# cloudflare/circl

Hardware: NVIDIA B200
Metric: ML-KEM-768 encaps/sec (higher is better)
Workload: dtype int16

## Files before the change

### circl_b200/csrc/api.cu

```cuda
#include <sched.h>
#include <stdarg.h>
#include <stdlib.h>
#include <string.h>

#include <algorithm>

#include "../../include/circl_b200.h"
#include "common.cuh"
#include "context.h"

#include <sys/mman.h>

namespace cb200 {

static thread_local char g_err[512] = "";
void set_error(const char* fmt, ...) {
  va_list ap;
  va_start(ap, fmt);
  vsnprintf(g_err, sizeof g_err, fmt, ap);
  va_end(ap);
}

Runtime& rt() {
  static Runtime* r = new Runtime;
  return *r;
}

static thread_local Dev* t_dev = nullptr;
static thread_local WorkSet* t_ws3 = nullptr;
static thread_local cudaStream_t t_stream = nullptr;

Dev& ctx() {
  if (!t_dev) {
    fprintf(stderr, "cb200: internal error: no device bound to this thread\n");
    abort();
  }
  return *t_dev;
}
WorkSet& wset(int slot) {
  if (slot >= 0 && slot < Dev::kSlots) return ctx().staging[slot];
  if (!t_ws3) {
    fprintf(stderr, "cb200: internal error: no work set bound to this thread\n");
    abort();
  }
  return *t_ws3;
}
bool profiling_on() { return rt().profiling; }

static const char* kKernelNames[KID_COUNT] = {
    "kyber_ntt", "kyber_invntt", "kyber_dot", "kyber_elementwise",
    "mlkem_hash_ek", "mlkem_g", "mlkem_sample", "mlkem_encrypt",
    "dil_ntt", "dil_invntt", "dil_dot", "dil_elementwise",
    "mldsa_expand_key", "mldsa_mu_rhoprime", "mldsa_mask", "mldsa_w", "mldsa_challenge", "mldsa_response",
    "mldsa_compact", "x25519", "hybrid_glue", "keccak_f1600", "sampler", "mlkem_sample_fix"};
const char* kernel_name(int id) { return (id >= 0 && id < KID_COUNT) ? kKernelNames[id] : "?"; }

KernelScope::KernelScope(int id_, cudaStream_t st_) : st(st_), id(id_) {
  Runtime& r = rt();
  r.launches.fetch_add(1, std::memory_order_relaxed);
  if (r.profiling) {
    cudaEventCreate(&a);
    cudaEventRecord(a, st);
  }
}
KernelScope::~KernelScope() {
  if (!a) return;
  Runtime& r = rt();
  cudaEvent_t b;
  cudaEventCreate(&b);
  cudaEventRecord(b, st);
  std::lock_guard<std::mutex> lock(r.prof_mu);
  r.prof.push_back(ProfRec{id, a, b});
}

int require_ready() {
  if (!rt().ready) {
    set_error("cb200: not initialised (call cb200_init or cb200_init_devices; there is no CPU fallback)");
    return CB200_ERR_NOT_INIT;
  }
  return 0;
}

bool is_device_ptr(const void* p, int* device) {
  if (!p) return false;
  cudaPointerAttributes a;
  if (cudaPointerGetAttributes(&a, p) != cudaSuccess) {
    cudaGetLastError();
// ... 45 lines not shown
  return 0;
}

int ensure_pinned(size_t bytes, void** out) {
  Dev& c = ctx();
  if (c.pinned_bytes < bytes) {
    if (c.pinned) CB200_CUDA(cudaFreeHost(c.pinned));
    c.pinned = nullptr;
    c.pinned_bytes = 0;
    CB200_CUDA(cudaHostAlloc(&c.pinned, bytes, cudaHostAllocDefault));
    c.pinned_bytes = bytes;
  }
  *out = c.pinned;
  return 0;
}

int ensure_smem_attr(const void* func, int bytes) {
  Dev& c = ctx();
  std::lock_guard<std::mutex> lock(c.attr_mu);
  if (c.attr_done.count(func)) return 0;
  CB200_CUDA(cudaFuncSetAttribute(func, cudaFuncAttributeMaxDynamicSharedMemorySize, bytes));
  c.attr_done.insert(func);
  return 0;
}

static int wset_create(WorkSet& w) {
  CB200_CUDA(cudaEventCreateWithFlags(&w.ev_fork, cudaEventDisableTiming));
  for (int l = 0; l < 2; l++) {
    CB200_CUDA(cudaStreamCreateWithFlags(&w.lane[l], cudaStreamNonBlocking));
    CB200_CUDA(cudaEventCreateWithFlags(&w.ev_join[l], cudaEventDisableTiming));
  }
  CB200_CUDA(cudaStreamCreateWithFlags(&w.copy, cudaStreamNonBlocking));
  CB200_CUDA(cudaEventCreateWithFlags(&w.ev_copy, cudaEventDisableTiming));
  CB200_CUDA(cudaMalloc(&w.small, 256));
  CB200_CUDA(cudaHostAlloc(&w.pin, 64, cudaHostAllocDefault));
  return 0;
}
static void wset_destroy(WorkSet& w) {
  for (int l = 0; l < 2; l++) {
    if (w.fix[l]) cudaFree(w.fix[l]);
    w.fix[l] = nullptr;
    w.fix_bytes[l] = 0;
    if (w.work[l]) cudaFree(w.work[l]);
    w.work[l] = nullptr;
    w.work_bytes[l] = 0;
    if (w.lane[l]) cudaStreamDestroy(w.lane[l]);
    if (w.ev_join[l]) cudaEventDestroy(w.ev_join[l]);
    w.lane[l] = nullptr;
    w.ev_join[l] = nullptr;
  }
  if (w.ev_fork) cudaEventDestroy(w.ev_fork);
  w.ev_fork = nullptr;
  if (w.copy) cudaStreamDestroy(w.copy);
  if (w.ev_copy) cudaEventDestroy(w.ev_copy);
  w.copy = nullptr;
  w.ev_copy = nullptr;
  if (w.small) cudaFree(w.small);
  if (w.pin) cudaFreeHost(w.pin);
  w.small = w.pin = nullptr;
}

static bool local_cpus(int device, cpu_set_t* out) {
  char id[32] = "";
  if (cudaDeviceGetPCIBusId(id, sizeof id, device) != cudaSuccess) {
    cudaGetLastError();
    return false;
  }
  for (char* p = id; *p; p++) *p = (char)tolower(*p);
  char path[128];
  snprintf(path, sizeof path, "/sys/bus/pci/devices/%s/local_cpulist", id);
  FILE* f = fopen(path, "r");
  if (!f) return false;
  char line[1024] = "";
  const bool got = fgets(line, sizeof line, f) != nullptr;
  fclose(f);
  if (!got) return false;
  cpu_set_t allowed;
  CPU_ZERO(&allowed);
  if (sched_getaffinity(0, sizeof allowed, &allowed) != 0) return false;
  CPU_ZERO(out);
  int n = 0;
  for (char* tok = strtok(line, ",\n"); tok; tok = strtok(nullptr, ",\n")) {
    int lo = 0, hi = 0;
    const int k = sscanf(tok, "%d-%d", &lo, &hi);
    if (k < 1) continue;
    if (k == 1) hi = lo;
    for (int c = lo; c <= hi && c < CPU_SETSIZE; c++)
      if (CPU_ISSET(c, &allowed)) {
        CPU_SET(c, out);
// ... 643 lines not shown
```

### circl_b200/csrc/context.h

```cpp
#pragma once
#include <cuda_runtime.h>
#include <stddef.h>
#include <stdint.h>

#include <atomic>
#include <condition_variable>
#include <deque>
#include <functional>
#include <map>
#include <memory>
#include <mutex>
#include <set>
#include <string>
#include <thread>
#include <vector>

#include "launch.h"

namespace cb200 {

struct ProfRec {
  int id;
  cudaEvent_t a, b;
};

struct WorkSet {
  void* work[2] = {nullptr, nullptr};
  size_t work_bytes[2] = {0, 0};
  cudaStream_t lane[2] = {nullptr, nullptr};
  cudaEvent_t ev_fork = nullptr, ev_join[2] = {nullptr, nullptr};
  cudaStream_t copy = nullptr;
  cudaEvent_t ev_copy = nullptr;
  void* fix[2] = {nullptr, nullptr};
  size_t fix_bytes[2] = {0, 0};
  void* small = nullptr;
  void* pin = nullptr;
  std::mutex mu;
};

struct Dev {
  int device = -1;
  int sm_count = 148;
  void* kyber_tw = nullptr;
  void* dil_tw = nullptr;
  void* x25519_table = nullptr;
  static constexpr int kSlots = 4;
  cudaStream_t pipe[kSlots] = {};
  cudaStream_t h2d = nullptr, d2h = nullptr;
  cudaEvent_t ev_in[kSlots] = {}, ev_k[kSlots] = {}, ev_out[kSlots] = {};
  void* scratch[kSlots] = {};
  size_t scratch_bytes[kSlots] = {};
  WorkSet staging[kSlots];
  void* pinned = nullptr;
  size_t pinned_bytes = 0;
  std::mutex sets_mu;
  std::map<cudaStream_t, std::unique_ptr<WorkSet>> sets;
  std::mutex attr_mu;
  std::set<const void*> attr_done;
  std::thread worker;
  std::mutex q_mu;
  std::condition_variable q_cv;
  std::deque<std::function<void()>> q;
  bool stop = false;
};

struct Runtime {
  std::vector<std::unique_ptr<Dev>> devs;
  std::atomic<bool> ready{false};
  std::atomic<uint64_t> launches{0};
  std::atomic<unsigned> next_dev{0};
  bool profiling = false;
  std::vector<ProfRec> prof;
  std::mutex prof_mu;
  std::mutex init_mu;
};
Runtime& rt();

enum KernelId {
  KID_KYBER_NTT = 0, KID_KYBER_INVNTT, KID_KYBER_DOT, KID_KYBER_EW,
  KID_MLKEM_HASH_EK, KID_MLKEM_G, KID_MLKEM_SAMPLE, KID_MLKEM_ENCRYPT,
  KID_DIL_NTT, KID_DIL_INVNTT, KID_DIL_DOT, KID_DIL_EW,
  KID_MLDSA_EXPAND, KID_MLDSA_MU, KID_MLDSA_MASK, KID_MLDSA_W, KID_MLDSA_CHALLENGE, KID_MLDSA_RESPONSE,
  KID_MLDSA_COMPACT, KID_X25519, KID_HYBRID_GLUE, KID_KECCAK, KID_SAMPLER, KID_MLKEM_SAMPLE_FIX, KID_COUNT
};
const char* kernel_name(int id);

Dev& ctx();
constexpr int kDevSlot = Dev::kSlots;
constexpr int kLevel1 = 8;
WorkSet& wset(int slot);
bool profiling_on();

struct KernelScope {
  cudaStream_t st;
  int id;
  cudaEvent_t a = nullptr;
  KernelScope(int id, cudaStream_t st);
  ~KernelScope();
};
int require_ready();
bool is_device_ptr(const void* p, int* device = nullptr);
int ensure_scratch(int slot, size_t bytes);
int ensure_work(int slot, size_t bytes, void** out);
int ensure_pinned(size_t bytes, void** out);
int ensure_fix(int slot, int lane, size_t bytes, cudaStream_t st, void** out);
int ensure_smem_attr(const void* func, int bytes);
inline void count_launch(uint64_t n = 1) { rt().launches.fetch_add(n, std::memory_order_relaxed); }

struct DeviceCall {
  int rc = 0;
  cudaStream_t st = nullptr;
  Dev* dev = nullptr;
  WorkSet* ws = nullptr;
  explicit DeviceCall(const void* any_device_buffer);
  ~DeviceCall();
  DeviceCall(const DeviceCall&) = delete;
// ... 37 lines not shown
```

### circl_b200/csrc/mlkem.cu

```cuda
#include <stdlib.h>
#include <string.h>

#include <algorithm>

#include "../../include/circl_b200.h"
#include "context.h"
#include "mlkem_internal.h"
#include "keccak.cuh"
#include "kyber.cuh"

namespace cb200 {
namespace mlkem {

using kyber::N;
using kyber::Q;

template <int K>
struct Params {
  static constexpr int k = K;
  static constexpr int du = (K == 4) ? 11 : 10;
  static constexpr int dv = (K == 4) ? 5 : 4;
  static constexpr int ek_bytes = 384 * K + 32;
  static constexpr int ct_bytes = 32 * (du * K + dv);
  static constexpr int eta1 = (K == 2) ? 3 : 2;
// ... 75 lines not shown
  }
  return wp;
}

__device__ __forceinline__ uint32_t prmt_sx(uint32_t a, uint32_t b, uint32_t sel) {
  uint32_t d;
  asm("prmt.b32 %0, %1, %2, %3;" : "=r"(d) : "r"(a), "r"(b), "r"(sel));
  return d;
}
__device__ __forceinline__ void cbd2_words(uint32_t t, uint32_t (&w)[4]) {
  const uint32_t d = (t & 0x55555555u) + ((t >> 1) & 0x55555555u);
  const uint32_t ae = d & 0x03030303u, be = (d >> 2) & 0x03030303u;
  const uint32_t ao = (d >> 4) & 0x03030303u, bo = (d >> 6) & 0x03030303u;
  const uint32_t ce = ((ae | 0x80808080u) - be) ^ 0x80808080u;
  const uint32_t co = ((ao | 0x80808080u) - bo) ^ 0x80808080u;
  w[0] = prmt_sx(ce, co, 0xc480);
  w[1] = prmt_sx(ce, co, 0xd591);
  w[2] = prmt_sx(ce, co, 0xe6a2);
  w[3] = prmt_sx(ce, co, 0xf7b3);
}
__device__ __forceinline__ void cbd2_store(const uint64_t (&a)[25], int16_t* __restrict__ dst) {
  uint4* out = reinterpret_cast<uint4*>(dst);
#pragma unroll
  for (int i = 0; i < 16; i++) {
    uint32_t lo[4], hi[4];
    cbd2_words((uint32_t)a[i], lo);
    cbd2_words((uint32_t)(a[i] >> 32), hi);
    out[2 * i] = make_uint4(lo[0], lo[1], lo[2], lo[3]);
    out[2 * i + 1] = make_uint4(hi[0], hi[1], hi[2], hi[3]);
  }
}

constexpr size_t kSub = 8192;
constexpr int kRowWords = 129;
constexpr int kSampleSmem = 128 * kRowWords * 4;

__device__ __forceinline__ void cbd3_store(const uint64_t (&w)[24], int16_t* __restrict__ dst) {
  uint4* out = reinterpret_cast<uint4*>(dst);
#pragma unroll
  for (int g = 0; g < 8; g++) {
    const uint64_t w0 = w[3 * g], w1 = w[3 * g + 1], w2 = w[3 * g + 2];
    uint64_t t[4];
    t[0] = w0;
    t[1] = (w0 >> 48) | (w1 << 16);
    t[2] = (w1 >> 32) | (w2 << 32);
    t[3] = w2 >> 16;
#pragma unroll
    for (int q = 0; q < 4; q++) {
      const uint64_t x = t[q];
      uint64_t d = x & 0x249249249249ull;
      d += (x >> 1) & 0x249249249249ull;
      d += (x >> 2) & 0x249249249249ull;
      uint32_t c[4];
#pragma unroll
      for (int j = 0; j < 4; j++) {
        const int c0 = (int)((d >> (12 * j)) & 7) - (int)((d >> (12 * j + 3)) & 7);
        const int c1 = (int)((d >> (12 * j + 6)) & 7) - (int)((d >> (12 * j + 9)) & 7);
        c[j] = ((uint32_t)c0 & 0xffffu) | ((uint32_t)c1 << 16);
      }
      out[4 * g + q] = make_uint4(c[0], c[1], c[2], c[3]);
    }
  }
}

__device__ __forceinline__ void uniform_stream(uint64_t (&a)[25], uint32_t* row_words) {
  int16_t* row = reinterpret_cast<int16_t*>(row_words);
// ... 320 lines not shown
    t[5] = ((b >> 28) | (c << 4)) & 0xfff;
    t[6] = (c >> 8) & 0xfff;
    t[7] = c >> 20;
#pragma unroll
    for (int j = 0; j < 8; j++) bad |= (t[j] >= (uint32_t)Q);
#pragma unroll
    for (int j = 0; j < 4; j++) aw[4 * g + j] = t[2 * j] | (t[2 * j + 1] << 16);
  }
  return bad;
}

__device__ __forceinline__ uint32_t unpack12_half(const uint32_t (&w)[8], uint32_t (&aw)[8]) {
  uint32_t bad = 0;
#pragma unroll
  for (int g = 0; g < 2; g++) {
    const uint32_t a = w[3 * g], b = w[3 * g + 1], c = w[3 * g + 2];
    uint32_t t[8];
    t[0] = a & 0xfff;
    t[1] = (a >> 12) & 0xfff;
    t[2] = ((a >> 24) | (b << 8)) & 0xfff;
    t[3] = (b >> 4) & 0xfff;
    t[4] = (b >> 16) & 0xfff;
    t[5] = ((b >> 28) | (c << 4)) & 0xfff;
    t[6] = (c >> 8) & 0xfff;
    t[7] = c >> 20;
#pragma unroll
    for (int j = 0; j < 8; j++) bad |= (t[j] >= (uint32_t)Q);
#pragma unroll
    for (int j = 0; j < 4; j++) aw[4 * g + j] = t[2 * j] | (t[2 * j + 1] << 16);
  }
  return bad;
}

template <int K, int THREADS, int MINB>
__global__ void __launch_bounds__(THREADS, MINB) encrypt_dp_kernel(
    const uint8_t* __restrict__ ek, size_t ek_stride, const int16_t* __restrict__ A, int a_shared,
    const int16_t* __restrict__ noise, const uint8_t* __restrict__ m, size_t n, uint8_t* __restrict__ ct,
    uint8_t* __restrict__ ss, uint8_t* __restrict__ status, const kyber::TwPair* __restrict__ tw, int lenient) {
  using P = Params<K>;
  using S = EncSmem<K, THREADS>;
  using namespace kyber;
  constexpr int OCTS = THREADS / 8;
  extern __shared__ __align__(16) uint32_t enc_smem[];
  uint32_t* ops_all = enc_smem;
  uint32_t* tiles = enc_smem + OCTS * S::op_words;
  TwPair* tws = reinterpret_cast<TwPair*>(tiles + OCTS * kPolyWords);
  const int lane = threadIdx.x & 31, warp = threadIdx.x >> 5, oct = lane >> 3, v = lane & 7;
  const unsigned octmask = 0xffu << (8 * oct);
  uint32_t* tile = tiles + (warp * 4 + oct) * kPolyWords;
  uint2* ops = reinterpret_cast<uint2*>(ops_all + (size_t)(warp * 4 + oct) * S::op_words) + v;

  for (int i = threadIdx.x; i < 128; i += THREADS) tws[i] = tw[128 + i];
  __syncthreads();
  const volatile TwLow* tabl = reinterpret_cast<const volatile TwLow*>(tws);
  const size_t base = ((size_t)blockIdx.x * (THREADS / 32) + warp) * 4;
  if (base >= n) return;
  const size_t op_raw = base + oct;
  const bool active = op_raw < n;
  const size_t op = active ? op_raw : n - 1;
  const uint8_t* ekp = ek + op * ek_stride;
  const uint32_t* Ap = reinterpret_cast<const uint32_t*>(A) + (a_shared ? 0 : op * K * K * (N / 2));
  const uint32_t* np = reinterpret_cast<const uint32_t*>(noise) + op * P::n_noise * (N / 2);
  uint8_t* ctp = ct + op * P::ct_bytes;

  int32_t r[32];

  {
    uint32_t nw[16];
#pragma unroll
    for (int q = 0; q < 16; q++) nw[q] = ldg_stream32(np + 8 * q + v);
#pragma unroll 1
    for (int j = 0; j < K; j++) {
#pragma unroll
      for (int q = 0; q < 16; q++) unpack2_lo(nw[q], r[2 * q], r[2 * q + 1]);
      if (j + 1 < K) {
#pragma unroll
        for (int q = 0; q < 16; q++) nw[q] = ldg_stream32(np + (j + 1) * (N / 2) + 8 * q + v);
      }
      fwd_pass_S_lo(r);
      store_S_lo(tile, v, r);
      __syncwarp();
      load_C_lo(tile, v, r);
      fwd_pass_C_lo_smem(r, tabl, v);
      __syncwarp();
#pragma unroll
      for (int q = 0; q < 8; q++) {
        const TwLow z = twl_at(tabl, 64 + 8 * q + v);
#pragma unroll
        for (int h = 0; h < 2; h++) {
          const int blk = 2 * q + h;
          const int32_t b0 = mont_mul_lo(r[2 * blk], kScaleZp, kScaleKk), b1 = mont_mul_lo(r[2 * blk + 1], kScaleZp, kScaleKk);
          int32_t zb1 = mont_mul_lo(b1, z.zp, z.kk);
          if (h) zb1 = -zb1;
          ops[(j * 16 + blk) * 8] = make_uint2(__byte_perm((uint32_t)b0, (uint32_t)zb1, 0x5140),
                                               __byte_perm((uint32_t)b1, (uint32_t)b0, 0x5140));
        }
      }
    }
  }
  __syncwarp();

  auto fetch = [&](int i, int h, int j, uint32_t (&raw)[8]) {
    if (i < K) {
      const uint4* p = reinterpret_cast<const uint4*>(Ap + (i * K + j) * (N / 2) + 16 * v + 8 * h);
      const uint4 x = __ldg(p), y = __ldg(p + 1);
      raw[0] = x.x, raw[1] = x.y, raw[2] = x.z, raw[3] = x.w, raw[4] = y.x, raw[5] = y.y, raw[6] = y.z, raw[7] = y.w;
    } else {
      const uint2* p = reinterpret_cast<const uint2*>(ekp + 384 * j + 48 * v + 24 * h);
      const uint2 x = __ldg(p), y = __ldg(p + 1), z = __ldg(p + 2);
      raw[0] = x.x, raw[1] = x.y, raw[2] = y.x, raw[3] = y.y, raw[4] = z.x, raw[5] = z.y;
    }
  };
  uint32_t bad = 0;
  uint32_t raw[K][8];
#pragma unroll
  for (int j = 0; j < K; j++) fetch(0, 0, j, raw[j]);
#pragma unroll 1
  for (int i = 0; i <= K; i++) {
    uint32_t ew[16];
#pragma unroll 1
    for (int h = 0; h < 2; h++) {
      int32_t p0l[8], p0h[8], p1l[8], p1h[8];
#pragma unroll
      for (int c = 0; c < 8; c++) p0l[c] = p0h[c] = p1l[c] = p1h[c] = 0;
      const int ni = h ? i + 1 : i, nh = h ^ 1;
#pragma unroll
      for (int j = 0; j < K; j++) {
        uint32_t aw[8];
        if (i < K) {
#pragma unroll
          for (int c = 0; c < 8; c++) aw[c] = raw[j][c];
        } else {
          const uint32_t b = unpack12_half(raw[j], aw);
          if (!lenient) bad |= b;
        }
        if (ni <= K) fetch(ni, nh, j, raw[j]);
        const uint2* oj = ops + (size_t)(j * 16 + 8 * h) * 8;
#pragma unroll
        for (int c = 0; c < 8; c++) {
          const uint2 w = oj[c * 8];
          p0l[c] = (int32_t)dp2a_lo_uu(aw[c], w.x, (uint32_t)p0l[c]);
          p0h[c] = dp2a_hi_us(aw[c], w.x, p0h[c]);
          p1l[c] = (int32_t)dp2a_lo_uu(aw[c], w.y, (uint32_t)p1l[c]);
          p1h[c] = dp2a_hi_us(aw[c], w.y, p1h[c]);
        }
      }
      if (h == 0) {
#pragma unroll
        for (int c = 0; c < 8; c++) {
          r[2 * c] = mont_red_lo(p0l[c] + p0h[c] * 256);
          r[2 * c + 1] = mont_red_lo(p1l[c] + p1h[c] * 256);
        }
        const uint32_t* e = np + (K + i) * (N / 2);
#pragma unroll
        for (int q = 0; q < 16; q++) ew[q] = __ldg(e + 8 * q + v);
      } else {
#pragma unroll
        for (int c = 0; c < 8; c++) {
          r[16 + 2 * c] = mont_red_lo(p0l[c] + p0h[c] * 256);
          r[16 + 2 * c + 1] = mont_red_lo(p1l[c] + p1h[c] * 256);
        }
      }
    }
    inv_pass_C_lo(r, tabl, v);
    store_C_lo(tile, v, r);
    __syncwarp();
    load_S_lo(tile, v, r);
    inv_pass_S_lo<false>(r, v);
    __syncwarp();
    {
      const uint32_t* mw = reinterpret_cast<const uint32_t*>(m + 32 * op);
#pragma unroll
      for (int s = 0; s < 16; s++) {
        int32_t e0, e1;
        unpack2_lo(ew[s], e0, e1);
        r[2 * s] += e0;
        r[2 * s + 1] += e1;
        if (i == K) {
          const uint32_t word = __ldg(mw + (s >> 1));
          const uint32_t bits = (word >> (16 * (s & 1) + 2 * v)) & 3;
          r[2 * s] += (bits & 1) ? (Q + 1) / 2 : 0;
          r[2 * s + 1] += (bits & 2) ? (Q + 1) / 2 : 0;
        }
      }
    }
    store_S_lo(tile, v, r);
    __syncwarp();
    load_C_lo(tile, v, r);
    __syncwarp();
    bad = __any_sync(octmask, bad) ? 1u : 0u;
    if (active) {
      if (i < K)
        compress_any_store_C<P::du, true>(r, reinterpret_cast<uint32_t*>(ctp + i * 32 * P::du) + v * P::du);
      else if (!bad)
        compress_any_store_C<P::dv, true>(r, reinterpret_cast<uint32_t*>(ctp + K * 32 * P::du) + v * P::dv);
    }
  }
  if (active) {
    if (bad) {
      uint32_t* c32 = reinterpret_cast<uint32_t*>(ctp);
      for (int w = v; w < P::ct_bytes / 4; w += 8) c32[w] = 0;
      if (ss) reinterpret_cast<uint32_t*>(ss + 32 * op)[v] = 0;
    }
    if (status && v == 0 && !lenient) status[op] = (uint8_t)bad;
  }
}

constexpr int kEncDpThreads = 64;
template <int K, int MINB>
static int launch_encrypt_v(const uint8_t* ek, size_t ek_stride, const int16_t* A, int a_shared, const int16_t* noise,
                            const uint8_t* m, size_t n, uint8_t* ct, uint8_t* ss, uint8_t* status, int lenient,
                            cudaStream_t st) {
  using S = EncSmem<K, kEncDpThreads>;
  if (int arc = ensure_smem_attr((const void*)encrypt_dp_kernel<K, kEncDpThreads, MINB>, S::bytes)) return arc;
  KernelScope ks(KID_MLKEM_ENCRYPT, st);
  constexpr int per_cta = kEncDpThreads / 8;
  encrypt_dp_kernel<K, kEncDpThreads, MINB><<<(unsigned)((n + per_cta - 1) / per_cta), kEncDpThreads, S::bytes, st>>>(
      ek, ek_stride, A, a_shared, noise, m, n, ct, ss, status, (const kyber::TwPair*)ctx().kyber_tw, lenient);
  return 0;
}
template <int K>
static int launch_encrypt(const uint8_t* ek, size_t ek_stride, const int16_t* A, int a_shared, const int16_t* noise,
                          const uint8_t* m, size_t n, uint8_t* ct, uint8_t* ss, uint8_t* status, int lenient,
                          cudaStream_t st) {
  return launch_encrypt_v<K, (K == 4 ? 6 : 7)>(ek, ek_stride, A, a_shared, noise, m, n, ct, ss, status, lenient, st);
}


template <int D, bool LOW = false>
__device__ __forceinline__ void decompress_C(const uint32_t* __restrict__ src, int32_t (&r)[32]) {
  uint32_t w[D + 1];
#pragma unroll
  for (int i = 0; i < D; i++) w[i] = __ldg(src + i);
  w[D] = 0;
#pragma unroll
  for (int i = 0; i < 32; i++) {
    const int bit = D * i, wi = bit >> 5, sh = bit & 31;
    uint32_t t = w[wi] >> sh;
    if (sh + D > 32) t |= w[wi + 1] << (32 - sh);
    t &= (1u << D) - 1;
    const uint32_t x = ((1u << (D - 1)) + t * (uint32_t)Q) >> D;
    r[i] = (int32_t)(LOW ? x : x << 16);
  }
}

template <int K, int THREADS, int MINB>
__global__ void __launch_bounds__(THREADS, MINB) decrypt_dp_kernel(const uint8_t* __restrict__ dk, size_t dk_stride,
                                                                   const uint8_t* __restrict__ ct, size_t n,
                                                                   uint8_t* __restrict__ mprime,
                                                                   const kyber::TwPair* __restrict__ tw) {
  using P = Params<K>;
  using S = EncSmem<K, THREADS>;
  using namespace kyber;
  constexpr int OCTS = THREADS / 8;
  extern __shared__ __align__(16) uint32_t enc_smem[];
  uint32_t* ops_all = enc_smem;
  uint32_t* tiles = enc_smem + OCTS * S::op_words;
  TwPair* tws = reinterpret_cast<TwPair*>(tiles + OCTS * kPolyWords);
  const int lane = threadIdx.x & 31, warp = threadIdx.x >> 5, oct = lane >> 3, v = lane & 7;
  const unsigned octmask = 0xffu << (8 * oct);
// ... 656 lines not shown
    r3_kdf_kernel<K><<<(unsigned)((n + 127) / 128), 128, 0, st>>>(in, ct2, kbar, key + 384 * K + P::ek_bytes + 32, key_stride,
                                                                  n, ss);
  }
  CB200_CUDA(cudaGetLastError());
  return 0;
}

struct Work {
  uint64_t* h;
  uint64_t* r;
  int16_t* A;
  int16_t* noise;
};


template <int K>
static int encaps_device(const uint8_t* ek, size_t ek_stride, const uint8_t* seeds, uint8_t* ct, uint8_t* ss,
                         uint8_t* status, size_t n, cudaStream_t st, int slot, uint8_t* push_ct = nullptr,
                         uint8_t* push_ss = nullptr) {
  using P = Params<K>;
  Dev& c = ctx();
  WorkSet& ws = wset(slot);
  const bool shared = (ek_stride == 0);
  const size_t nkeys = shared ? 1 : n;
  const size_t sub = n < kSub ? n : kSub;
  const size_t subkeys = shared ? 1 : sub;
  size_t off = 0;
  auto take = [&](size_t bytes) {
    size_t o = off;
    off += (bytes + 255) & ~(size_t)255;
    return o;
  };
  const size_t o_h = take(nkeys * 32), o_r = take(n * 32);
  size_t o_A[2], o_n[2];
  o_A[0] = take(subkeys * K * K * 512);
  o_A[1] = shared ? o_A[0] : take(subkeys * K * K * 512);
  o_n[0] = take(sub * P::n_noise * 512);
  o_n[1] = take(sub * P::n_noise * 512);
  void* base = nullptr;
  int rc = ensure_work(slot, off, &base);
  if (rc) return rc;
  uint64_t* h = (uint64_t*)((char*)base + o_h);
  uint64_t* r = (uint64_t*)((char*)base + o_r);

  if (int arc = ensure_smem_attr((const void*)sample_kernel<K>, kSampleSmem)) return arc;
  {
    KernelScope ks(KID_MLKEM_HASH_EK, st);
    hash_ek_kernel<K><<<(unsigned)((nkeys + 127) / 128), 128, 0, st>>>(ek, ek_stride, nkeys, h);
  }
  {
    KernelScope ks(KID_MLKEM_G, st);
    g_kernel<<<(unsigned)((n + 127) / 128), 128, 0, st>>>(seeds, (const uint8_t*)h, shared ? 0 : 32, n, ss, r);
  }
  if (shared)
    if (int src = launch_sample<K>(slot, 0, st, ek + 384 * K, 0, 1, r, 0, (int16_t*)((char*)base + o_A[0]),
                                   (int16_t*)((char*)base + o_n[0]), 1, P::n_noise, 4, K))
      return src;
  CB200_CUDA(cudaEventRecord(ws.ev_fork, st));
  for (int l = 0; l < 2; l++) CB200_CUDA(cudaStreamWaitEvent(ws.lane[l], ws.ev_fork, 0));
  int l = 0;
  for (size_t first = 0; first < n; first += sub, l ^= 1) {
    cudaStream_t ls = profiling_on() ? st : ws.lane[l];
    int16_t* A = (int16_t*)((char*)base + o_A[l]);
    int16_t* noise = (int16_t*)((char*)base + o_n[l]);
    const size_t cnt = (n - first < sub) ? n - first : sub;
    const size_t keys_here = shared ? 0 : cnt;
    if (int src = launch_sample<K>(slot, l, ls, ek + 384 * K + (shared ? 0 : first * ek_stride), ek_stride, keys_here,
                                   r + 4 * first, cnt, A, noise, 1, P::n_noise, 4, K))
      return src;
    if (int erc = launch_encrypt<K>(ek + (shared ? 0 : first * ek_stride), ek_stride, A, shared ? 1 : 0, noise,
                                    seeds + 32 * first, cnt, ct + first * P::ct_bytes, ss + 32 * first,
                                    status ? status + first : nullptr, 0, ls))
      return erc;
    if (push_ct || push_ss) {
      CB200_CUDA(cudaEventRecord(ws.ev_copy, ls));
      CB200_CUDA(cudaStreamWaitEvent(ws.copy, ws.ev_copy, 0));
      if (push_ct)
        CB200_CUDA(cudaMemcpyAsync(push_ct + first * P::ct_bytes, ct + first * P::ct_bytes, cnt * (size_t)P::ct_bytes,
                                   cudaMemcpyDefault, ws.copy));
      if (push_ss) CB200_CUDA(cudaMemcpyAsync(push_ss + 32 * first, ss + 32 * first, cnt * 32, cudaMemcpyDefault, ws.copy));
    }
  }
  if (push_ct || push_ss) {
    CB200_CUDA(cudaEventRecord(ws.ev_copy, ws.copy));
    CB200_CUDA(cudaStreamWaitEvent(st, ws.ev_copy, 0));
  }
  for (int q = 0; q < 2; q++) {
    CB200_CUDA(cudaEventRecord(ws.ev_join[q], ws.lane[q]));
    CB200_CUDA(cudaStreamWaitEvent(st, ws.ev_join[q], 0));
  }
  CB200_CUDA(cudaGetLastError());
  return 0;
}

static int encaps_any(int k, const uint8_t* ek, size_t ek_stride, const uint8_t* seeds, uint8_t* ct, uint8_t* ss,
                      uint8_t* status, size_t n, cudaStream_t st, int slot, uint8_t* push_ct = nullptr,
                      uint8_t* push_ss = nullptr) {
  return k == 2   ? encaps_device<2>(ek, ek_stride, seeds, ct, ss, status, n, st, slot, push_ct, push_ss)
         : k == 3 ? encaps_device<3>(ek, ek_stride, seeds, ct, ss, status, n, st, slot, push_ct, push_ss)
// ... 530 lines not shown
```

Measured before the change: 57.80 million.

## Overlap chunked hash/G with sampling and add opt-in fused encaps kernel

Default non-shared encaps now runs hash_ek and G kernels in chunks on an auxiliary stream, recording an event per chunk. Each encrypt lane waits only on the chunks it needs, so sampling and encryption can begin before all hashing finishes. The change also adds an env-gated fused kernel that does sampling, noise PRF and encryption in shared memory, and moves the encrypt body into a templated function shared by both paths. It adds stream and event overhead and more launches.

```diff
diff --git a/circl_b200/csrc/api.cu b/circl_b200/csrc/api.cu
--- a/circl_b200/csrc/api.cu
+++ b/circl_b200/csrc/api.cu
@@ -52,7 +52,8 @@
     "mlkem_hash_ek", "mlkem_g", "mlkem_sample", "mlkem_encrypt",
     "dil_ntt", "dil_invntt", "dil_dot", "dil_elementwise",
     "mldsa_expand_key", "mldsa_mu_rhoprime", "mldsa_mask", "mldsa_w", "mldsa_challenge", "mldsa_response",
-    "mldsa_compact", "x25519", "hybrid_glue", "keccak_f1600", "sampler", "mlkem_sample_fix"};
+    "mldsa_compact", "x25519", "hybrid_glue", "keccak_f1600", "sampler", "mlkem_sample_fix",
+    "mlkem_encaps"};
 const char* kernel_name(int id) { return (id >= 0 && id < KID_COUNT) ? kKernelNames[id] : "?"; }
 
 KernelScope::KernelScope(int id_, cudaStream_t st_) : st(st_), id(id_) {
@@ -164,6 +165,8 @@
   }
   CB200_CUDA(cudaStreamCreateWithFlags(&w.copy, cudaStreamNonBlocking));
   CB200_CUDA(cudaEventCreateWithFlags(&w.ev_copy, cudaEventDisableTiming));
+  CB200_CUDA(cudaStreamCreateWithFlags(&w.aux, cudaStreamNonBlocking));
+  for (cudaEvent_t& e : w.ev_aux) CB200_CUDA(cudaEventCreateWithFlags(&e, cudaEventDisableTiming));
   CB200_CUDA(cudaMalloc(&w.small, 256));
   CB200_CUDA(cudaHostAlloc(&w.pin, 64, cudaHostAllocDefault));
   return 0;
@@ -187,6 +190,12 @@
   if (w.ev_copy) cudaEventDestroy(w.ev_copy);
   w.copy = nullptr;
   w.ev_copy = nullptr;
+  if (w.aux) cudaStreamDestroy(w.aux);
+  w.aux = nullptr;
+  for (cudaEvent_t& e : w.ev_aux) {
+    if (e) cudaEventDestroy(e);
+    e = nullptr;
+  }
   if (w.small) cudaFree(w.small);
   if (w.pin) cudaFreeHost(w.pin);
   w.small = w.pin = nullptr;
diff --git a/circl_b200/csrc/context.h b/circl_b200/csrc/context.h
--- a/circl_b200/csrc/context.h
+++ b/circl_b200/csrc/context.h
@@ -30,6 +30,9 @@
   cudaStream_t lane[2] = {nullptr, nullptr};
   cudaEvent_t ev_fork = nullptr, ev_join[2] = {nullptr, nullptr};
   cudaStream_t copy = nullptr;
+  static constexpr int kAuxEvents = 16;
+  cudaStream_t aux = nullptr;
+  cudaEvent_t ev_aux[kAuxEvents] = {};
   cudaEvent_t ev_copy = nullptr;
   void* fix[2] = {nullptr, nullptr};
   size_t fix_bytes[2] = {0, 0};
@@ -81,7 +84,8 @@
   KID_MLKEM_HASH_EK, KID_MLKEM_G, KID_MLKEM_SAMPLE, KID_MLKEM_ENCRYPT,
   KID_DIL_NTT, KID_DIL_INVNTT, KID_DIL_DOT, KID_DIL_EW,
   KID_MLDSA_EXPAND, KID_MLDSA_MU, KID_MLDSA_MASK, KID_MLDSA_W, KID_MLDSA_CHALLENGE, KID_MLDSA_RESPONSE,
-  KID_MLDSA_COMPACT, KID_X25519, KID_HYBRID_GLUE, KID_KECCAK, KID_SAMPLER, KID_MLKEM_SAMPLE_FIX, KID_COUNT
+  KID_MLDSA_COMPACT, KID_X25519, KID_HYBRID_GLUE, KID_KECCAK, KID_SAMPLER, KID_MLKEM_SAMPLE_FIX, KID_MLKEM_ENCAPS,
+  KID_COUNT
 };
 const char* kernel_name(int id);
 
diff --git a/circl_b200/csrc/mlkem.cu b/circl_b200/csrc/mlkem.cu
--- a/circl_b200/csrc/mlkem.cu
+++ b/circl_b200/csrc/mlkem.cu
@@ -131,6 +131,7 @@
 }
 
 constexpr size_t kSub = 8192;
+constexpr size_t kHashChunk = 1u << 16;
 constexpr int kRowWords = 129;
 constexpr int kSampleSmem = 128 * kRowWords * 4;
 
@@ -517,6 +518,170 @@
   return bad;
 }
 
+template <int K>
+struct EncGlobalSrc {
+  const uint32_t* __restrict__ Ap;
+  const uint32_t* __restrict__ np;
+  int v;
+  __device__ __forceinline__ void operands_built() const {}
+  __device__ __forceinline__ void noise_r(int p, uint32_t (&w)[16]) const {
+#pragma unroll
+    for (int q = 0; q < 16; q++) w[q] = ldg_stream32(np + p * (N / 2) + 8 * q + v);
+  }
+  __device__ __forceinline__ void noise_e(int p, uint32_t (&w)[16]) const {
+#pragma unroll
+    for (int q = 0; q < 16; q++) w[q] = __ldg(np + p * (N / 2) + 8 * q + v);
+  }
+  __device__ __forceinline__ void a_half(int i, int j, int h, uint32_t (&raw)[8]) const {
+    const uint4* p = reinterpret_cast<const uint4*>(Ap + (i * K + j) * (N / 2) + 16 * v + 8 * h);
+    const uint4 x = __ldg(p), y = __ldg(p + 1);
+    raw[0] = x.x, raw[1] = x.y, raw[2] = x.z, raw[3] = x.w, raw[4] = y.x, raw[5] = y.y, raw[6] = y.z, raw[7] = y.w;
+  }
+};
+
+template <int K, class Src>
+__device__ __forceinline__ void encrypt_octet(const Src& src, const uint8_t* __restrict__ ekp, const uint8_t* __restrict__ m,
+                                              size_t op, bool active, uint8_t* __restrict__ ctp, uint8_t* __restrict__ ss,
+                                              uint8_t* __restrict__ status, int lenient, unsigned octmask, int v,
+                                              uint32_t* tile, uint2* ops, const volatile kyber::TwLow* tabl) {
+  using P = Params<K>;
+  using namespace kyber;
+  int32_t r[32];
+
+  {
+    uint32_t nw[16];
+    src.noise_r(0, nw);
+#pragma unroll 1
+    for (int j = 0; j < K; j++) {
+#pragma unroll
+      for (int q = 0; q < 16; q++) unpack2_lo(nw[q], r[2 * q], r[2 * q + 1]);
+      if (j + 1 < K) src.noise_r(j + 1, nw);
+      fwd_pass_S_lo(r);
+      store_S_lo(tile, v, r);
+      __syncwarp();
+      load_C_lo(tile, v, r);
+      fwd_pass_C_lo_smem(r, tabl, v);
+      __syncwarp();
+#pragma unroll
+      for (int q = 0; q < 8; q++) {
+        const TwLow z = twl_at(tabl, 64 + 8 * q + v);
+#pragma unroll
+        for (int h = 0; h < 2; h++) {
+          const int blk = 2 * q + h;
+          const int32_t b0 = mont_mul_lo(r[2 * blk], kScaleZp, kScaleKk), b1 = mont_mul_lo(r[2 * blk + 1], kScaleZp, kScaleKk);
+          int32_t zb1 = mont_mul_lo(b1, z.zp, z.kk);
+          if (h) zb1 = -zb1;
+          ops[(j * 16 + blk) * 8] = make_uint2(__byte_perm((uint32_t)b0, (uint32_t)zb1, 0x5140),
+                                               __byte_perm((uint32_t)b1, (uint32_t)b0, 0x5140));
+        }
+      }
+    }
+  }
+  __syncwarp();
+  src.operands_built();
+
+  auto fetch = [&](int i, int h, int j, uint32_t (&raw)[8]) {
+    if (i < K) {
+      src.a_half(i, j, h, raw);
+    } else {
+      const uint2* p = reinterpret_cast<const uint2*>(ekp + 384 * j + 48 * v + 24 * h);
+      const uint2 x = __ldg(p), y = __ldg(p + 1), z = __ldg(p + 2);
+      raw[0] = x.x, raw[1] = x.y, raw[2] = y.x, raw[3] = y.y, raw[4] = z.x, raw[5] = z.y;
+    }
+  };
+  uint32_t bad = 0;
+  uint32_t raw[K][8];
+#pragma unroll
+  for (int j = 0; j < K; j++) fetch(0, 0, j, raw[j]);
+#pragma unroll 1
+  for (int i = 0; i <= K; i++) {
+    uint32_t ew[16];
+#pragma unroll 1
+    for (int h = 0; h < 2; h++) {
+      int32_t p0l[8], p0h[8], p1l[8], p1h[8];
+#pragma unroll
+      for (int c = 0; c < 8; c++) p0l[c] = p0h[c] = p1l[c] = p1h[c] = 0;
+      const int ni = h ? i + 1 : i, nh = h ^ 1;
+#pragma unroll
+      for (int j = 0; j < K; j++) {
+        uint32_t aw[8];
+        if (i < K) {
+#pragma unroll
+          for (int c = 0; c < 8; c++) aw[c] = raw[j][c];
+        } else {
+          const uint32_t b = unpack12_half(raw[j], aw);
+          if (!lenient) bad |= b;
+        }
+        if (ni <= K) fetch(ni, nh, j, raw[j]);
+        const uint2* oj = ops + (size_t)(j * 16 + 8 * h) * 8;
+#pragma unroll
+        for (int c = 0; c < 8; c++) {
+          const uint2 w = oj[c * 8];
+          p0l[c] = (int32_t)dp2a_lo_uu(aw[c], w.x, (uint32_t)p0l[c]);
+          p0h[c] = dp2a_hi_us(aw[c], w.x, p0h[c]);
+          p1l[c] = (int32_t)dp2a_lo_uu(aw[c], w.y, (uint32_t)p1l[c]);
+          p1h[c] = dp2a_hi_us(aw[c], w.y, p1h[c]);
+        }
+      }
+      if (h == 0) {
+#pragma unroll
+        for (int c = 0; c < 8; c++) {
+          r[2 * c] = mont_red_lo(p0l[c] + p0h[c] * 256);
+          r[2 * c + 1] = mont_red_lo(p1l[c] + p1h[c] * 256);
+        }
+        src.noise_e(K + i, ew);
+      } else {
+#pragma unroll
+        for (int c = 0; c < 8; c++) {
+          r[16 + 2 * c] = mont_red_lo(p0l[c] + p0h[c] * 256);
+          r[16 + 2 * c + 1] = mont_red_lo(p1l[c] + p1h[c] * 256);
+        }
+      }
+    }
+    inv_pass_C_lo(r, tabl, v);
+    store_C_lo(tile, v, r);
+    __syncwarp();
+    load_S_lo(tile, v, r);
+    inv_pass_S_lo<false>(r, v);
+    __syncwarp();
+    {
+      const uint32_t* mw = reinterpret_cast<const uint32_t*>(m + 32 * op);
+#pragma unroll
+      for (int s = 0; s < 16; s++) {
+        int32_t e0, e1;
+        unpack2_lo(ew[s], e0, e1);
+        r[2 * s] += e0;
+        r[2 * s + 1] += e1;
+        if (i == K) {
+          const uint32_t word = __ldg(mw + (s >> 1));
+          const uint32_t bits = (word >> (16 * (s & 1) + 2 * v)) & 3;
+          r[2 * s] += (bits & 1) ? (Q + 1) / 2 : 0;
+          r[2 * s + 1] += (bits & 2) ? (Q + 1) / 2 : 0;
+        }
+      }
+    }
+    store_S_lo(tile, v, r);
+    __syncwarp();
+    load_C_lo(tile, v, r);
+    __syncwarp();
+    bad = __any_sync(octmask, bad) ? 1u : 0u;
+    if (active) {
+      if (i < K)
+        compress_any_store_C<P::du, true>(r, reinterpret_cast<uint32_t*>(ctp + i * 32 * P::du) + v * P::du);
+      else if (!bad)
+        compress_any_store_C<P::dv, true>(r, reinterpret_cast<uint32_t*>(ctp + K * 32 * P::du) + v * P::dv);
+    }
+  }
+  if (active) {
+    if (bad) {
+      uint32_t* c32 = reinterpret_cast<uint32_t*>(ctp);
+      for (int w = v; w < P::ct_bytes / 4; w += 8) c32[w] = 0;
+      if (ss) reinterpret_cast<uint32_t*>(ss + 32 * op)[v] = 0;
+    }
+    if (status && v == 0 && !lenient) status[op] = (uint8_t)bad;
+  }
+}
+
 template <int K, int THREADS, int MINB>
 __global__ void __launch_bounds__(THREADS, MINB) encrypt_dp_kernel(
     const uint8_t* __restrict__ ek, size_t ek_stride, const int16_t* __restrict__ A, int a_shared,
@@ -543,153 +708,12 @@
   const size_t op_raw = base + oct;
   const bool active = op_raw < n;
   const size_t op = active ? op_raw : n - 1;
-  const uint8_t* ekp = ek + op * ek_stride;
-  const uint32_t* Ap = reinterpret_cast<const uint32_t*>(A) + (a_shared ? 0 : op * K * K * (N / 2));
-  const uint32_t* np = reinterpret_cast<const uint32_t*>(noise) + op * P::n_noise * (N / 2);
-  uint8_t* ctp = ct + op * P::ct_bytes;
-
-  int32_t r[32];
-
-  {
-    uint32_t nw[16];
-#pragma unroll
-    for (int q = 0; q < 16; q++) nw[q] = ldg_stream32(np + 8 * q + v);
-#pragma unroll 1
-    for (int j = 0; j < K; j++) {
-#pragma unroll
-      for (int q = 0; q < 16; q++) unpack2_lo(nw[q], r[2 * q], r[2 * q + 1]);
-      if (j + 1 < K) {
-#pragma unroll
-        for (int q = 0; q < 16; q++) nw[q] = ldg_stream32(np + (j + 1) * (N / 2) + 8 * q + v);
-      }
-      fwd_pass_S_lo(r);
-      store_S_lo(tile, v, r);
-      __syncwarp();
-      load_C_lo(tile, v, r);
-      fwd_pass_C_lo_smem(r, tabl, v);
-      __syncwarp();
-#pragma unroll
-      for (int q = 0; q < 8; q++) {
-        const TwLow z = twl_at(tabl, 64 + 8 * q + v);
-#pragma unroll
-        for (int h = 0; h < 2; h++) {
-          const int blk = 2 * q + h;
-          const int32_t b0 = mont_mul_lo(r[2 * blk], kScaleZp, kScaleKk), b1 = mont_mul_lo(r[2 * blk + 1], kScaleZp, kScaleKk);
-          int32_t zb1 = mont_mul_lo(b1, z.zp, z.kk);
-          if (h) zb1 = -zb1;
-          ops[(j * 16 + blk) * 8] = make_uint2(__byte_perm((uint32_t)b0, (uint32_t)zb1, 0x5140),
-                                               __byte_perm((uint32_t)b1, (uint32_t)b0, 0x5140));
-        }
-      }
-    }
-  }
-  __syncwarp();
-
-  auto fetch = [&](int i, int h, int j, uint32_t (&raw)[8]) {
-    if (i < K) {
-      const uint4* p = reinterpret_cast<const uint4*>(Ap + (i * K + j) * (N / 2) + 16 * v + 8 * h);
-      const uint4 x = __ldg(p), y = __ldg(p + 1);
-      raw[0] = x.x, raw[1] = x.y, raw[2] = x.z, raw[3] = x.w, raw[4] = y.x, raw[5] = y.y, raw[6] = y.z, raw[7] = y.w;
-    } else {
-      const uint2* p = reinterpret_cast<const uint2*>(ekp + 384 * j + 48 * v + 24 * h);
-      const uint2 x = __ldg(p), y = __ldg(p + 1), z = __ldg(p + 2);
-      raw[0] = x.x, raw[1] = x.y, raw[2] = y.x, raw[3] = y.y, raw[4] = z.x, raw[5] = z.y;
-    }
-  };
-  uint32_t bad = 0;
-  uint32_t raw[K][8];
-#pragma unroll
-  for (int j = 0; j < K; j++) fetch(0, 0, j, raw[j]);
-#pragma unroll 1
-  for (int i = 0; i <= K; i++) {
-    uint32_t ew[16];
-#pragma unroll 1
-    for (int h = 0; h < 2; h++) {
-      int32_t p0l[8], p0h[8], p1l[8], p1h[8];
-#pragma unroll
-      for (int c = 0; c < 8; c++) p0l[c] = p0h[c] = p1l[c] = p1h[c] = 0;
-      const int ni = h ? i + 1 : i, nh = h ^ 1;
-#pragma unroll
-      for (int j = 0; j < K; j++) {
-        uint32_t aw[8];
-        if (i < K) {
-#pragma unroll
-          for (int c = 0; c < 8; c++) aw[c] = raw[j][c];
-        } else {
-          const uint32_t b = unpack12_half(raw[j], aw);
-          if (!lenient) bad |= b;
-        }
-        if (ni <= K) fetch(ni, nh, j, raw[j]);
-        const uint2* oj = ops + (size_t)(j * 16 + 8 * h) * 8;
-#pragma unroll
-        for (int c = 0; c < 8; c++) {
-          const uint2 w = oj[c * 8];
-          p0l[c] = (int32_t)dp2a_lo_uu(aw[c], w.x, (uint32_t)p0l[c]);
-          p0h[c] = dp2a_hi_us(aw[c], w.x, p0h[c]);
-          p1l[c] = (int32_t)dp2a_lo_uu(aw[c], w.y, (uint32_t)p1l[c]);
-          p1h[c] = dp2a_hi_us(aw[c], w.y, p1h[c]);
-        }
-      }
-      if (h == 0) {
-#pragma unroll
-        for (int c = 0; c < 8; c++) {
-          r[2 * c] = mont_red_lo(p0l[c] + p0h[c] * 256);
-          r[2 * c + 1] = mont_red_lo(p1l[c] + p1h[c] * 256);
-        }
-        const uint32_t* e = np + (K + i) * (N / 2);
-#pragma unroll
-        for (int q = 0; q < 16; q++) ew[q] = __ldg(e + 8 * q + v);
-      } else {
-#pragma unroll
-        for (int c = 0; c < 8; c++) {
-          r[16 + 2 * c] = mont_red_lo(p0l[c] + p0h[c] * 256);
-          r[16 + 2 * c + 1] = mont_red_lo(p1l[c] + p1h[c] * 256);
-        }
-      }
-    }
-    inv_pass_C_lo(r, tabl, v);
-    store_C_lo(tile, v, r);
-    __syncwarp();
-    load_S_lo(tile, v, r);
-    inv_pass_S_lo<false>(r, v);
-    __syncwarp();
-    {
-      const uint32_t* mw = reinterpret_cast<const uint32_t*>(m + 32 * op);
-#pragma unroll
-      for (int s = 0; s < 16; s++) {
-        int32_t e0, e1;
-        unpack2_lo(ew[s], e0, e1);
-        r[2 * s] += e0;
-        r[2 * s + 1] += e1;
-        if (i == K) {
-          const uint32_t word = __ldg(mw + (s >> 1));
-          const uint32_t bits = (word >> (16 * (s & 1) + 2 * v)) & 3;
-          r[2 * s] += (bits & 1) ? (Q + 1) / 2 : 0;
-          r[2 * s + 1] += (bits & 2) ? (Q + 1) / 2 : 0;
-        }
-      }
-    }
-    store_S_lo(tile, v, r);
-    __syncwarp();
-    load_C_lo(tile, v, r);
-    __syncwarp();
-    bad = __any_sync(octmask, bad) ? 1u : 0u;
-    if (active) {
-      if (i < K)
-        compress_any_store_C<P::du, true>(r, reinterpret_cast<uint32_t*>(ctp + i * 32 * P::du) + v * P::du);
-      else if (!bad)
-        compress_any_store_C<P::dv, true>(r, reinterpret_cast<uint32_t*>(ctp + K * 32 * P::du) + v * P::dv);
-    }
-  }
-  if (active) {
-    if (bad) {
-      uint32_t* c32 = reinterpret_cast<uint32_t*>(ctp);
-      for (int w = v; w < P::ct_bytes / 4; w += 8) c32[w] = 0;
-      if (ss) reinterpret_cast<uint32_t*>(ss + 32 * op)[v] = 0;
-    }
-    if (status && v == 0 && !lenient) status[op] = (uint8_t)bad;
-  }
-}
+  const EncGlobalSrc<K> src{reinterpret_cast<const uint32_t*>(A) + (a_shared ? 0 : op * K * K * (N / 2)),
+                            reinterpret_cast<const uint32_t*>(noise) + op * P::n_noise * (N / 2), v};
+  encrypt_octet<K>(src, ek + op * ek_stride, m, op, active, ct + op * P::ct_bytes, ss, status, lenient, octmask, v, tile,
+                   ops, tabl);
+}
+
 
 constexpr int kEncDpThreads = 64;
 template <int K, int MINB>
@@ -711,6 +735,196 @@
   return launch_encrypt_v<K, (K == 4 ? 6 : 7)>(ek, ek_stride, A, a_shared, noise, m, n, ct, ss, status, lenient, st);
 }
 
+
+constexpr int kFusedOps = 8;
+constexpr int kFusedThreads = 96;
+constexpr int kFusedMinBlocks = 3;
+constexpr size_t kFusedPushPiece = 1u << 16;
+
+template <int K>
+struct FusedSmem {
+  static constexpr int mat = kFusedOps * K * K;
+  static constexpr int noise = kFusedOps * Params<K>::n_noise;
+  static constexpr int noise_lanes = kFusedThreads - mat;
+  static constexpr int rows = mat * kRowWords;
+  static constexpr int prf = noise * 32;
+  static constexpr int op_words = EncSmem<K, 8 * kFusedOps>::op_words;
+  static constexpr int ops = kFusedOps * op_words;
+  static constexpr int words = rows + prf + ops + kFusedOps * kyber::kPolyWords + 256;
+  static constexpr int bytes = words * 4;
+  static_assert(noise <= 3 * noise_lanes && noise > 2 * noise_lanes, "three PRF blocks per noise lane");
+  static_assert(Params<K>::eta1 == 2, "raw PRF storage assumes CBD_2 for every noise polynomial");
+};
+struct ShortStream {
+  uint64_t a[25];
+  uint32_t row, wp;
+};
+
+template <int K>
+struct EncSharedSrc {
+  const uint32_t* rows;
+  const uint32_t* prf;
+  int v;
+  uint32_t sel;
+  __device__ __forceinline__ void noise(int p, uint32_t (&w)[16]) const {
+    const uint32_t* s = prf + 32 * p + (v >> 2);
+#pragma unroll
+    for (int k = 0; k < 4; k++) {
+      const uint32_t g = __byte_perm(__byte_perm(s[8 * k], s[8 * k + 2], sel), __byte_perm(s[8 * k + 4], s[8 * k + 6], sel),
+                                     0x5410);
+      uint32_t c[4];
+      cbd2_words(g, c);
+#pragma unroll
+      for (int e = 0; e < 4; e++) w[4 * k + e] = c[e];
+    }
+  }
+  __device__ __forceinline__ void operands_built() const { asm volatile("bar.sync 1, %0;" ::"n"(kFusedThreads) : "memory"); }
+  __device__ __forceinline__ void noise_r(int p, uint32_t (&w)[16]) const { noise(p, w); }
+  __device__ __forceinline__ void noise_e(int p, uint32_t (&w)[16]) const { noise(p, w); }
+  __device__ __forceinline__ void a_half(int i, int j, int h, uint32_t (&raw)[8]) const {
+    const uint32_t* p = rows + (i * K + j) * kRowWords + 16 * v + 8 * h;
+#pragma unroll
+    for (int c = 0; c < 8; c++) raw[c] = p[c];
+  }
+};
+
+template <int K>
+__global__ void __launch_bounds__(kFusedThreads, kFusedMinBlocks) encaps_fused_kernel(
+    const uint8_t* __restrict__ ek, size_t ek_stride, const uint64_t* __restrict__ r, const uint8_t* __restrict__ m,
+    size_t n, uint8_t* __restrict__ ct, uint8_t* __restrict__ ss, uint8_t* __restrict__ status,
+    const kyber::TwPair* __restrict__ tw, unsigned long long* __restrict__ next_tile, ShortStream* __restrict__ spill) {
+  using P = Params<K>;
+  using S = FusedSmem<K>;
+  using namespace kyber;
+  extern __shared__ __align__(16) uint32_t fsm[];
+  uint32_t* rows = fsm;
+  uint32_t* prf = rows + S::rows;
+  uint32_t* ops_all = prf + S::prf;
+  uint32_t* tiles = ops_all + S::ops;
+  TwPair* tws = reinterpret_cast<TwPair*>(tiles + kFusedOps * kPolyWords);
+  ShortStream* shorts = spill + (size_t)blockIdx.x * S::mat;
+  __shared__ unsigned int n_short;
+  __shared__ unsigned long long s_tile;
+  const int t = threadIdx.x, lane = t & 31, v = lane & 7;
+  for (int i = t; i < 128; i += kFusedThreads) tws[i] = tw[128 + i];
+  if (t == 0) {
+    n_short = 0;
+    s_tile = atomicAdd(next_tile, 1ull);
+  }
+  __syncthreads();
+  const volatile TwLow* tabl = reinterpret_cast<const volatile TwLow*>(tws);
+
+  const bool mat = t < S::mat;
+  const int mop = t / (K * K), ij = t % (K * K);
+  const int nl = t - S::mat;
+  const size_t n_tiles = (n + kFusedOps - 1) / kFusedOps;
+  for (;;) {
+    const size_t tile = s_tile;
+    if (tile >= n_tiles) break;
+    const size_t first = tile * kFusedOps;
+    {
+      uint64_t a[25];
+      keccak::zero(a);
+      uint32_t wp = 0, wend = 0;
+      if (mat) {
+        const uint8_t* rho = ek + std::min(first + mop, n - 1) * ek_stride + 384 * K;
+#pragma unroll
+        for (int w = 0; w < 4; w++) a[w] = keccak::ld64(rho + 8 * w);
+        a[4] = (uint64_t)(ij / K) | ((uint64_t)(ij % K) << 8) | (0x1full << 16);
+        a[20] = 0x8000000000000000ull;
+        wp = smem_u32(rows + t * kRowWords);
+        wend = wp + 2 * N;
+      }
+#pragma unroll 1
+      for (int b = 0; b < 3; b++) {
+        const int ns = nl + b * S::noise_lanes;
+        if (!mat) {
+          keccak::zero(a);
+          const size_t op = std::min(first + ns / P::n_noise, n - 1);
+#pragma unroll
+          for (int w = 0; w < 4; w++) a[w] = r[4 * op + w];
+          a[4] = (uint64_t)(ns % P::n_noise) | (0x1full << 8);
+          a[16] = 0x8000000000000000ull;
+        }
+        keccak::f1600(a);
+        if (mat) {
+          wp = b < 2 ? reject_block<false>(a, wp, wend) : reject_block<true>(a, wp, wend);
+        } else if (ns < S::noise) {
+          uint4* dst = reinterpret_cast<uint4*>(prf + 32 * ns);
+#pragma unroll
+          for (int q = 0; q < 8; q++)
+            dst[q] = make_uint4((uint32_t)a[2 * q], (uint32_t)(a[2 * q] >> 32), (uint32_t)a[2 * q + 1],
+                                (uint32_t)(a[2 * q + 1] >> 32));
+        }
+      }
+      if (mat && wp < wend && first + mop < n) {
+        ShortStream& e = shorts[atomicAdd(&n_short, 1u)];
+        e.row = (uint32_t)t;
+        e.wp = wp;
+#pragma unroll
+        for (int w = 0; w < 25; w++) e.a[w] = a[w];
+      }
+    }
+    __syncthreads();
+    if (t < 8 * kFusedOps) {
+      const int o = t >> 3;
+      const size_t op_raw = first + o;
+      const bool active = op_raw < n;
+      const size_t op = active ? op_raw : n - 1;
+      const EncSharedSrc<K> src{rows + o * K * K * kRowWords, prf + o * P::n_noise * 32, v,
+                                (uint32_t)(v & 3) | ((4u + (v & 3)) << 4)};
+      encrypt_octet<K>(src, ek + op * ek_stride, m, op, active, ct + op * P::ct_bytes, ss, status, 0,
+                       0xffu << (8 * (o & 3)), v, tiles + o * kPolyWords,
+                       reinterpret_cast<uint2*>(ops_all + o * S::op_words) + v, tabl);
+    } else {
+      const unsigned int cnt = n_short;
+      for (unsigned int x = lane; x < cnt; x += 32) {
+        uint64_t a[25];
+#pragma unroll
+        for (int w = 0; w < 25; w++) a[w] = shorts[x].a[w];
+        uint32_t wp = shorts[x].wp;
+        const uint32_t wend = smem_u32(rows + shorts[x].row * kRowWords) + 2 * N;
+        do {
+          keccak::f1600(a);
+          wp = reject_block<true>(a, wp, wend);
+        } while (wp < wend);
+      }
+      if (lane == 0) {
+        n_short = 0;
+        s_tile = atomicAdd(next_tile, 1ull);
+      }
+      asm volatile("bar.sync 1, %0;" ::"n"(kFusedThreads) : "memory");
+    }
+    __syncthreads();
+  }
+}
+
+template <int K>
+static size_t fused_scratch_bytes(int ctas) {
+  return 256 + (size_t)ctas * FusedSmem<K>::mat * sizeof(ShortStream);
+}
+template <int K>
+static int fused_ctas() {
+  static const int per_sm = [] {
+    int b = 0;
+    cudaOccupancyMaxActiveBlocksPerMultiprocessor(&b, encaps_fused_kernel<K>, kFusedThreads, FusedSmem<K>::bytes);
+    return b > 0 ? b : 1;
+  }();
+  return ctx().sm_count * per_sm;
+}
+template <int K>
+static int launch_encaps_fused(const uint8_t* ek, size_t ek_stride, const uint64_t* r, const uint8_t* m, size_t n,
+                               uint8_t* ct, uint8_t* ss, uint8_t* status, void* scratch, cudaStream_t st) {
+  using S = FusedSmem<K>;
+  if (int arc = ensure_smem_attr((const void*)encaps_fused_kernel<K>, S::bytes)) return arc;
+  const size_t tiles = (n + kFusedOps - 1) / kFusedOps;
+  CB200_CUDA(cudaMemsetAsync(scratch, 0, sizeof(unsigned long long), st));
+  KernelScope ks(KID_MLKEM_ENCAPS, st);
+  encaps_fused_kernel<K><<<(unsigned)std::min<size_t>(tiles, (size_t)fused_ctas<K>()), kFusedThreads, S::bytes, st>>>(
+      ek, ek_stride, r, m, n, ct, ss, status, (const kyber::TwPair*)ctx().kyber_tw, (unsigned long long*)scratch,
+      (ShortStream*)((char*)scratch + 256));
+  return 0;
+}
 
 template <int D, bool LOW = false>
 __device__ __forceinline__ void decompress_C(const uint32_t* __restrict__ src, int32_t (&r)[32]) {
@@ -1433,6 +1647,44 @@
     return o;
   };
   const size_t o_h = take(nkeys * 32), o_r = take(n * 32);
+  const char* path = getenv("CB200_MLKEM_ENCAPS");
+  if constexpr (K == 3) if (!shared && path && !strcmp(path, "fused")) {
+    const size_t o_fs = take(fused_scratch_bytes<K>(fused_ctas<K>()));
+    void* base = nullptr;
+    if (int rc = ensure_work(slot, off, &base)) return rc;
+    uint64_t* h = (uint64_t*)((char*)base + o_h);
+    uint64_t* r = (uint64_t*)((char*)base + o_r);
+    {
+      KernelScope ks(KID_MLKEM_HASH_EK, st);
+      hash_ek_kernel<K><<<(unsigned)((n + 127) / 128), 128, 0, st>>>(ek, ek_stride, n, h);
+    }
+    {
+      KernelScope ks(KID_MLKEM_G, st);
+      g_kernel<<<(unsigned)((n + 127) / 128), 128, 0, st>>>(seeds, (const uint8_t*)h, 32, n, ss, r);
+    }
+    const size_t piece = (push_ct || push_ss) ? kFusedPushPiece : n;
+    for (size_t first = 0; first < n; first += piece) {
+      const size_t cnt = std::min(piece, n - first);
+      if (int frc = launch_encaps_fused<K>(ek + first * ek_stride, ek_stride, r + 4 * first, seeds + 32 * first, cnt,
+                                           ct + first * P::ct_bytes, ss + 32 * first, status ? status + first : nullptr,
+                                           (char*)base + o_fs, st))
+        return frc;
+      if (push_ct || push_ss) {
+        CB200_CUDA(cudaEventRecord(ws.ev_copy, st));
+        CB200_CUDA(cudaStreamWaitEvent(ws.copy, ws.ev_copy, 0));
+        if (push_ct)
+          CB200_CUDA(cudaMemcpyAsync(push_ct + first * P::ct_bytes, ct + first * P::ct_bytes, cnt * (size_t)P::ct_bytes,
+                                     cudaMemcpyDefault, ws.copy));
+        if (push_ss) CB200_CUDA(cudaMemcpyAsync(push_ss + 32 * first, ss + 32 * first, cnt * 32, cudaMemcpyDefault, ws.copy));
+      }
+    }
+    if (push_ct || push_ss) {
+      CB200_CUDA(cudaEventRecord(ws.ev_copy, ws.copy));
+      CB200_CUDA(cudaStreamWaitEvent(st, ws.ev_copy, 0));
+    }
+    CB200_CUDA(cudaGetLastError());
+    return 0;
+  }
   size_t o_A[2], o_n[2];
   o_A[0] = take(subkeys * K * K * 512);
   o_A[1] = shared ? o_A[0] : take(subkeys * K * K * 512);
@@ -1445,19 +1697,40 @@
   uint64_t* r = (uint64_t*)((char*)base + o_r);
 
   if (int arc = ensure_smem_attr((const void*)sample_kernel<K>, kSampleSmem)) return arc;
-  {
-    KernelScope ks(KID_MLKEM_HASH_EK, st);
-    hash_ek_kernel<K><<<(unsigned)((nkeys + 127) / 128), 128, 0, st>>>(ek, ek_stride, nkeys, h);
-  }
-  {
-    KernelScope ks(KID_MLKEM_G, st);
-    g_kernel<<<(unsigned)((n + 127) / 128), 128, 0, st>>>(seeds, (const uint8_t*)h, shared ? 0 : 32, n, ss, r);
+  const bool ahead = !shared && !profiling_on();
+  const size_t chunk = std::max<size_t>(kHashChunk, (n + WorkSet::kAuxEvents - 1) / WorkSet::kAuxEvents);
+  if (ahead) {
+    CB200_CUDA(cudaEventRecord(ws.ev_fork, st));
+    CB200_CUDA(cudaStreamWaitEvent(ws.aux, ws.ev_fork, 0));
+    for (size_t first = 0, c = 0; first < n; first += chunk, c++) {
+      const size_t cnt = std::min(chunk, n - first);
+      {
+        KernelScope ks(KID_MLKEM_HASH_EK, ws.aux);
+        hash_ek_kernel<K><<<(unsigned)((cnt + 127) / 128), 128, 0, ws.aux>>>(ek + first * ek_stride, ek_stride, cnt,
+                                                                            h + 4 * first);
+      }
+      {
+        KernelScope ks(KID_MLKEM_G, ws.aux);
+        g_kernel<<<(unsigned)((cnt + 127) / 128), 128, 0, ws.aux>>>(seeds + 32 * first, (const uint8_t*)(h + 4 * first),
+                                                                    32, cnt, ss + 32 * first, r + 4 * first);
+      }
+      CB200_CUDA(cudaEventRecord(ws.ev_aux[c], ws.aux));
+    }
+  } else {
+    {
+      KernelScope ks(KID_MLKEM_HASH_EK, st);
+      hash_ek_kernel<K><<<(unsigned)((nkeys + 127) / 128), 128, 0, st>>>(ek, ek_stride, nkeys, h);
+    }
+    {
+      KernelScope ks(KID_MLKEM_G, st);
+      g_kernel<<<(unsigned)((n + 127) / 128), 128, 0, st>>>(seeds, (const uint8_t*)h, shared ? 0 : 32, n, ss, r);
+    }
   }
   if (shared)
     if (int src = launch_sample<K>(slot, 0, st, ek + 384 * K, 0, 1, r, 0, (int16_t*)((char*)base + o_A[0]),
                                    (int16_t*)((char*)base + o_n[0]), 1, P::n_noise, 4, K))
       return src;
-  CB200_CUDA(cudaEventRecord(ws.ev_fork, st));
+  if (!ahead) CB200_CUDA(cudaEventRecord(ws.ev_fork, st));
   for (int l = 0; l < 2; l++) CB200_CUDA(cudaStreamWaitEvent(ws.lane[l], ws.ev_fork, 0));
   int l = 0;
   for (size_t first = 0; first < n; first += sub, l ^= 1) {
@@ -1466,6 +1739,10 @@
     int16_t* noise = (int16_t*)((char*)base + o_n[l]);
     const size_t cnt = (n - first < sub) ? n - first : sub;
     const size_t keys_here = shared ? 0 : cnt;
+    if (ahead) {
+      for (size_t c = first / chunk; c <= (first + cnt - 1) / chunk; c++)
+        CB200_CUDA(cudaStreamWaitEvent(ls, ws.ev_aux[c], 0));
+    }
     if (int src = launch_sample<K>(slot, l, ls, ek + 384 * K + (shared ? 0 : first * ek_stride), ek_stride, keys_here,
                                    r + 4 * first, cnt, A, noise, 1, P::n_noise, 4, K))
       return src;
```

Measured after the change: 57.16 million, median of 6. 0.989x the previous value.
